# IceTTTb/NopeSAC

Measured on AMD Instinct MI355X. Metric: image-pairs/sec (480x640, K=32 hyp), higher is better.
Workload: dtype bf16; 1 GPU; configs/inference_mp3d.yaml, 32 synthetic 480x640 pairs/GPU/step, ResNet-50 + pyramids in bfloat16, head GEMMs bf16 operands with f32 accumulate / residual stream / LayerNorm / softmax, K=32 matched planes forced (m mean 32.0), nq=50; pairs_per_gpu=32, global_batch=32, K=32, parallelism=pair-sharded dp1, rccl_ranks=1, batches_in_flight_per_gpu=4, hip_graph=False, steps_per_all_gather=8, routing_entries_loaded=45, routing_entries_measured_now=0, nonfinite_outputs=0

## Files before the change

nopesac_amd/csrc/conv_forms.h:

```cpp
#pragma once
#include <initializer_list>

#include "common.h"

namespace nps {

constexpr int P8_SK_MAX_TILES = 4096;

struct ConvCall {
    int x_dt, w_dt, out_dt;
    int B, H, W, Cin, Cout, KH, KW, stride, pad;
    long long x_cs, y_cs, r_cs;
    bool batched, has_residual, has_scale, has_bias;
    int act;
    bool aligned, entry;

    static long long fdiv(long long a, long long b) { return a / b - ((a % b != 0 && ((a < 0) != (b < 0))) ? 1 : 0); }
    long long OH() const { return fdiv(H + 2ll * pad - KH, stride) + 1; }
    long long OW() const { return fdiv(W + 2ll * pad - KW, stride) + 1; }
    long long M() const { return B * OH() * OW(); }
    long long K() const { return (long long)KH * KW * Cin; }
    long long tiles(int bm, int bn) const { return -fdiv(-M(), bm) * (Cout / bn); }
};

static inline bool conv_aligned(std::initializer_list<const void*> ptrs) {
    for (const void* q : ptrs)
        if ((uintptr_t)q % 16 != 0) return false;
    return true;
}

#define NPS_CHECK_CONV(name, expr)                  \
    do {                                            \
        const char* why__ = (expr);                 \
        NPS_CHECK_ARG(!why__, name ": %s", why__);  \
    } while (0)


static inline const char* conv_call_refusal(const ConvCall& c) {
    if (!(c.B > 0 && c.H > 0 && c.W > 0 && c.Cin > 0 && c.Cout > 0 && c.KH > 0 && c.KW > 0 && c.stride > 0 && c.pad >= 0)) return "bad dims";
    if (c.OH() <= 0 || c.OW() <= 0) return "empty output";
    if (c.out_dt != NPS_DT_F32 && c.out_dt != NPS_DT_BF16 && c.out_dt != NPS_DT_FP8) return "bad out_dt";
    if (c.x_cs < c.Cin || c.y_cs < c.Cout || (c.has_residual && c.r_cs < c.Cout)) return "channel stride smaller than channel count";
    if ((c.act & 0xff) > NPS_ACT_SIGMOID) return "bad act";
    return nullptr;
}

static inline const char* conv_dma_refusal(const ConvCall& c, int cout_tile) {
    const int eb = c.x_dt == NPS_DT_FP8 ? 1 : 2;
    if ((c.x_dt != NPS_DT_BF16 && c.x_dt != NPS_DT_FP8) || c.w_dt != c.x_dt || c.batched) return "needs bf16 (or fp8) x and w, shared weights";
    if (c.Cin % 64 != 0 || c.Cout % cout_tile != 0) return cout_tile == 256 ? "needs Cin % 64 == 0 and Cout % 256 == 0" : "needs Cin % 64 == 0 and Cout % 128 == 0";
    if (c.KH * c.KW > 32) return "more than 32 taps";
    if (c.x_cs % (16 / eb) != 0) return "x_cstride must be a multiple of 16 bytes";
    if (((long long)c.B * c.H * c.W + (long long)c.pad * c.W + c.pad) * c.x_cs * eb >= (1ll << 31)) return "input larger than 2 GB";
    return nullptr;
}

static inline const char* conv_idx24_refusal(const ConvCall& c) {
    if ((long long)c.B * c.H * c.W >= (1 << 23) || c.x_cs >= (1 << 24) || c.K() >= (1 << 24)) return "pixel count / strides beyond the 24-bit index math of this kernel";
    if (c.Cout * c.K() * 2 >= (1ll << 31)) return "weights larger than 2 GB";
    return nullptr;
}

static inline const char* conv_bfrag_refusal(const ConvCall& c) {
    if (const char* why = conv_dma_refusal(c, 128)) return why;
    if (c.act & ~(0xff | NPS_ACT_RES_AFTER)) return "unsupported act flags";
    if (c.entry && c.out_dt == NPS_DT_FP8 && (c.has_residual || c.y_cs % 8 != 0 || !c.aligned)) return "fp8 output needs no residual and 8-channel-aligned y / scale / bias";
    return nullptr;
}

static inline const char* conv_halo_refusal(const ConvCall& c) {
    if (const char* why = conv_bfrag_refusal(c)) return why;
    if (c.x_dt != NPS_DT_BF16 || c.out_dt != NPS_DT_BF16) return "bf16 only";
    if (c.KH != 3 || c.KW != 3 || c.stride != 1 || c.pad != 1) return "3x3 / stride 1 / pad 1 only";
    if (c.x_cs != c.Cin || c.y_cs != c.Cout) return "dense channels only";
    if (c.has_residual || !c.has_scale || !c.has_bias || (c.act & ~0xff)) return "y = act(conv * scale + bias) only: scale and bias, no residual";
    return nullptr;
}

static inline const char* conv_p8_refusal(const ConvCall& c) {
    if (const char* why = conv_dma_refusal(c, 256)) return why;
    if (c.x_dt != NPS_DT_BF16) return "bf16 only";
    if (const char* why = conv_idx24_refusal(c)) return why;
    if (c.act & ~(0xff | NPS_ACT_RES_AFTER)) return "unsupported act flags";
    if (c.out_dt != NPS_DT_F32 && c.out_dt != NPS_DT_BF16 && c.out_dt != NPS_DT_FP8) return "bad out_dt";
    const int al = c.out_dt == NPS_DT_F32 ? 4 : 8;
    if (c.has_residual && c.out_dt == NPS_DT_FP8) return "residual with fp8 output";
    if (!c.aligned || c.y_cs % al != 0 || (c.has_residual && c.r_cs % al != 0)) return "every buffer must be 16-byte aligned with 16-byte-aligned y / residual strides";
    if (c.entry && c.M() >= (1 << 23)) return "output pixel count beyond the 24-bit index math of this kernel";
    return nullptr;
}

static inline const char* conv_p8_sk_refusal(const ConvCall& c) {
    if (const char* why = conv_p8_refusal(c)) return why;
    if (c.tiles(256, 256) > P8_SK_MAX_TILES) return "more tiles than the stream-K workspace has arrival counters (use the plain kernel: nothing to balance)";
    return nullptr;
}

static inline const char* conv_p8n_refusal(const ConvCall& c) {
    if (const char* why = conv_dma_refusal(c, 128)) return why;
    if (c.x_dt != NPS_DT_BF16 || c.out_dt != NPS_DT_BF16 || c.has_residual) return "bf16 in / bf16 out, no residual";
    if (const char* why = conv_idx24_refusal(c)) return why;
    if (c.act != NPS_ACT_NONE && c.act != NPS_ACT_RELU && c.act != NPS_ACT_LEAKY) return "act must be none / ReLU / LeakyReLU (no residual forms)";
    if (!c.aligned || c.y_cs % 8 != 0) return "every buffer must be 16-byte aligned with y_cstride % 8 == 0";
    if ((c.M() + 256) * c.y_cs * 2 >= (1ll << 31)) return "output larger than 2 GB";
    return nullptr;
}

static inline const char* conv_p8n_split_refusal(const ConvCall& c, int splits) {
    if (const char* why = conv_p8n_refusal(c)) return why;
    if (splits < 2 || splits > c.Cin / 64 || splits > 16) return "2 <= splits <= min(Cin / 64, 16)";
    if (splits * c.M() * c.Cout * 4 >= (1ll << 31)) return "split-K workspace larger than 2 GB";
    return nullptr;
}


static inline bool conv_p8_sk_offered(const ConvCall& c) { return c.tiles(256, 256) <= 1024 && c.K() >= 512; }

static inline bool conv_p8n_tap_offered(const ConvCall& c) { return c.KH * c.KW > 1; }

static inline int conv_p8n_split_slices(const ConvCall& c) {
    const long long tiles = c.Cout % 128 == 0 ? c.tiles(256, 128) : 0;
    if (tiles == 0) return 0;
    long long s = ConvCall::fdiv(256, tiles);
    if (s > c.Cin / 64) s = c.Cin / 64;
    return (int)(s > 8 ? 8 : s);
}
static inline bool conv_p8n_split_offered(const ConvCall& c, int splits) { return c.K() >= 4096 && splits >= 2; }

}
```

nopesac_amd/csrc/conv_p8_tile.h:

```cpp
#pragma once
#include "conv_common.h"

namespace nps {

template <int K>
struct IC { static constexpr int value = K; };

typedef unsigned int u32x4 __attribute__((ext_vector_type(4)));

constexpr unsigned P8_OOB = 0xFFFFFF00u;

struct P8TileWalk {
    int xcd, slot, run_begin, run_end, stride;
    __device__ __forceinline__ explicit P8TileWalk(int units) {
        const int nx = (int)gridDim.x < 8 ? (int)gridDim.x : 8;
        xcd = blockIdx.x % 8; slot = blockIdx.x / 8;
        const int tq = units / nx, tr = units % nx;
        run_begin = xcd < tr ? xcd * (tq + 1) : tr * (tq + 1) + (xcd - tr) * tq;
        run_end = run_begin + tq + (xcd < tr ? 1 : 0);
        stride = ((int)gridDim.x - xcd + 7) / 8;
    }
};

__device__ __forceinline__ __amdgpu_buffer_rsrc_t p8_x_rsrc(const ConvParams& p) {
    const long long padb = ((long long)p.pad * p.W + p.pad) * p.x_cs * 2;
    return __builtin_amdgcn_make_buffer_rsrc((void*)((const char*)p.x - padb), 0, (int)(((long long)p.B * p.H * p.W * p.x_cs) * 2 + padb), 0x00020000);
}
__device__ __forceinline__ __amdgpu_buffer_rsrc_t p8_w_rsrc(const ConvParams& p) {
    return __builtin_amdgcn_make_buffer_rsrc((void*)p.w, 0, (int)((long long)p.N * p.K * 2), 0x00020000);
}
__device__ __forceinline__ __amdgpu_buffer_rsrc_t p8_rows_rsrc(const void* base, const ConvParams& p, long long cs, bool on = true) {
    return __builtin_amdgcn_make_buffer_rsrc((void*)base, 0, on ? (int)((((long long)p.M - 1) * cs + p.N) * 2) : 0, 0x00020000);
}

__device__ __forceinline__ void p8_divmod(int a, int d, float rcp, int& q, int& r) {
    q = (int)((float)a * rcp);
    r = a - __mul24(q, d);
    if (r < 0) { --q; r += d; }
    if (r >= d) { ++q; r -= d; }
}

template <int BK>
struct P8KCursor {
    int tap, kw, c0;
    unsigned tapoff, k0b;
    unsigned kw_step, kh_step;
    __device__ __forceinline__ explicit P8KCursor(const ConvParams& p)
        : kw_step((unsigned)p.x_cs * 2u), kh_step((unsigned)(p.W - p.KW) * (unsigned)p.x_cs * 2u) {}
    __device__ __forceinline__ void reset(int c_begin) {
        tap = 0; kw = 0; c0 = c_begin; tapoff = 0u; k0b = (unsigned)c_begin * 2u;
    }
    __device__ __forceinline__ void advance(const ConvParams& p) {
        if (p.force == 0) {
            k0b += BK * 2;
            c0 += BK;
            if (c0 >= p.Cin) {
                c0 = 0; ++tap; ++kw;
                tapoff += kw_step;
                if (kw == p.KW) { kw = 0; tapoff += kh_step; }
            }
        } else {
            ++tap; ++kw;
            k0b += (unsigned)p.Cin * 2u;
            tapoff += kw_step;
            if (kw == p.KW) { kw = 0; tapoff += kh_step; }
            if (tap == p.KH * p.KW) {
                tap = 0; kw = 0; tapoff = 0u;
                c0 += BK;
                k0b = (unsigned)c0 * 2u;
            }
        }
    }
    __device__ __forceinline__ void set_cursor(const ConvParams& p, int kt) {
        const int ntaps = p.KH * p.KW;
        int t, c;
        if (p.force == 0) { const int per = p.Cin / BK; t = kt / per; c = (kt - t * per) * BK; }
        else { const int cs = kt / ntaps; t = kt - cs * ntaps; c = cs * BK; }
        const int kh = t / p.KW;
        tap = t; kw = t - kh * p.KW; c0 = c;
        tapoff = (unsigned)(kh * p.W + kw) * (unsigned)p.x_cs * 2u;
        k0b = (unsigned)(t * p.Cin + c) * 2u;
    }
};

template <int BM, int ROWB, int TAB_OFF>
struct P8Rows {
    static_assert(BM == 256 && ROWB == 128, "two pixel halves of two 64-row DMA groups, 128-byte rows");
    unsigned coff[2][2], voff[2][2], mask[2][2];
    float rcp_rpb, rcp_ow;
    __device__ __forceinline__ void init(const ConvParams& p, int wave, int lane) {
        rcp_rpb = 1.0f / (float)p.rows_per_b; rcp_ow = 1.0f / (float)p.OW;
#pragma unroll
        for (int h = 0; h < 2; ++h)
#pragma unroll
            for (int j = 0; j < 2; ++j) {
                const int pr = j * 128 + h * 64 + wave * 8 + (lane >> 3);
                coff[h][j] = (unsigned)((lane & 7) ^ ((pr >> 1) & 7)) * 16u;
            }
    }
    __device__ __forceinline__ void set_tile(unsigned char* lds, const ConvParams& p, int m0, int tid, int wave, int lane) {
        uint2* rowtab = reinterpret_cast<uint2*>(lds + TAB_OFF);
        if (tid < BM) {
            const int m = m0 + tid;
            uint2 e = make_uint2(0u, 0u);
            if (m < p.M) {
                int b, rem, oh, ow;
                p8_divmod(m, p.rows_per_b, rcp_rpb, b, rem);
                p8_divmod(rem, p.OW, rcp_ow, oh, ow);
                const int ih0 = __mul24(oh, p.stride) - p.pad, iw0 = __mul24(ow, p.stride) - p.pad;
                const unsigned pix = __umul24(__umul24((unsigned)b, (unsigned)p.H) + (unsigned)(ih0 + p.pad), (unsigned)p.W) + (unsigned)(iw0 + p.pad);
                unsigned colbits = 0u;
                for (int kw = 0; kw < p.KW; ++kw) colbits |= ((unsigned)(iw0 + kw) < (unsigned)p.W ? 1u : 0u) << kw;
                unsigned mk = 0u;
                for (int kh = 0; kh < p.KH; ++kh)
                    if ((unsigned)(ih0 + kh) < (unsigned)p.H) mk |= colbits << __mul24(kh, p.KW);
                e = make_uint2(__umul24(pix, (unsigned)p.x_cs) * 2u, mk);
            }
            rowtab[tid] = e;
        }
        NPS_LDS_SYNC();
#pragma unroll
        for (int h = 0; h < 2; ++h)
#pragma unroll
            for (int j = 0; j < 2; ++j) {
                const uint2 e = rowtab[j * 128 + h * 64 + wave * 8 + (lane >> 3)];
                voff[h][j] = e.x + coff[h][j];
                mask[h][j] = e.y;
            }
    }
    template <int BK>
    __device__ __forceinline__ void stage_a(const __amdgpu_buffer_rsrc_t& xsrc, unsigned char* buf, int h, int wave, const P8KCursor<BK>& cur) const {
        const unsigned soff = cur.tapoff + (unsigned)cur.c0 * 2u;
#pragma unroll
        for (int j = 0; j < 2; ++j) {
            const unsigned vo = ((mask[h][j] >> cur.tap) & 1u) ? voff[h][j] : P8_OOB;
            __builtin_amdgcn_raw_ptr_buffer_load_lds(xsrc, (lptr_t)(buf + (j * 128 + h * 64 + wave * 8) * ROWB), 16, vo, soff, 0, 0);
        }
    }
};

}
```

nopesac_amd/csrc/conv_p8n.hip:

```cpp
#include "conv_forms.h"
#include "conv_p8_tile.h"

namespace nps {

constexpr int N8_BM = 256, N8_BN = 128, N8_BK = 64, N8_ROWB = 128;
constexpr int N8_A_BYTES = N8_BM * N8_ROWB, N8_B_BYTES = N8_BN * N8_ROWB, N8_STAGE = N8_A_BYTES + N8_B_BYTES;
constexpr int N8_NSTAGE = 3;
constexpr int N8_ELD16 = N8_BN + 8;
constexpr int N8_EPI_OFF = 2 * N8_STAGE;
constexpr int N8_TAB_OFF = N8_NSTAGE * N8_STAGE;
constexpr int N8_LDS = N8_TAB_OFF + N8_BM * 8;

struct N8EpiRegs {
    float sc[4][4], bs[4][4];
};

template <int ACT, bool SPLIT = false>
__global__ __launch_bounds__(512) void conv_igemm_p8n_kernel(const ConvParams p) {
#if defined(__HIP_DEVICE_COMPILE__)
    __shared__ __attribute__((aligned(1024))) unsigned char lds[N8_LDS];
    const int tid = threadIdx.x, lane = tid & 63;
    const int wave = __builtin_amdgcn_readfirstlane(tid >> 6);
    const int wr = wave >> 2, wc = wave & 3;

    const P8TileWalk walk(p.tiles_m * p.tiles_n * (SPLIT ? p.ksplit : 1));
    int tile = walk.run_begin + walk.slot;
    if (tile >= walk.run_end) return;

    const __amdgpu_buffer_rsrc_t xsrc = p8_x_rsrc(p), wsrc = p8_w_rsrc(p), ry = p8_rows_rsrc(p.y, p, p.y_cs);
    P8Rows<N8_BM, N8_ROWB, N8_TAB_OFF> rows;
    P8KCursor<N8_BK> kc(p);
    rows.init(p, wave, lane);
    unsigned b_voff[2], b_base[2];
#pragma unroll
    for (int j = 0; j < 2; ++j) {
        const int br = (wave * 2 + j) * 8 + (lane >> 3);
        b_base[j] = (__umul24((unsigned)br, (unsigned)p.K) + (unsigned)((lane & 7) ^ ((br >> 1) & 7)) * 8u) * 2u;
    }
    int m0 = 0, n0 = 0;
    const int ntaps = p.KH * p.KW;
    int nk = p.K / N8_BK;
    int ks = 0;
    auto set_tile = [&](int t) {
        int c_begin = 0;
        if constexpr (SPLIT) {
            const int tt = t / p.ksplit, ngroups = p.Cin / N8_BK;
            ks = t - tt * p.ksplit;
            c_begin = (ks * ngroups) / p.ksplit;
            nk = (((ks + 1) * ngroups) / p.ksplit - c_begin) * ntaps;
            c_begin *= N8_BK;
            t = tt;
        }
        m0 = (t / p.tiles_n) * N8_BM;
        n0 = (t % p.tiles_n) * N8_BN;
        rows.set_tile(lds, p, m0, tid, wave, lane);
        const unsigned nb = __umul24((unsigned)n0, (unsigned)p.K) * 2u;
#pragma unroll
        for (int j = 0; j < 2; ++j) b_voff[j] = b_base[j] + nb;
        kc.reset(c_begin);
    };
    auto stage_a = [&](unsigned char* buf, int h) { rows.stage_a(xsrc, buf, h, wave, kc); };
    auto stage_b = [&](unsigned char* buf) {
#pragma unroll
        for (int j = 0; j < 2; ++j)
            __builtin_amdgcn_raw_ptr_buffer_load_lds(wsrc, (lptr_t)(buf + N8_A_BYTES + ((wave * 2 + j) * 8) * N8_ROWB), 16, b_voff[j], kc.k0b, 0, 0);
    };
    auto stage_first = [&]() {
        stage_a(lds, 0); stage_b(lds); stage_a(lds, 1);
        kc.advance(p);
        if (nk > 1) {
            stage_a(lds + N8_STAGE, 0); stage_b(lds + N8_STAGE); stage_a(lds + N8_STAGE, 1);
            kc.advance(p);
        }
    };

    const int sw = (lane >> 1) & 7;
    const int a_row_off = (wr * 128 + (lane & 31)) * N8_ROWB;
    const int b_row_off = N8_A_BYTES + (wc * 32 + (lane & 31)) * N8_ROWB;
    int so[4];
#pragma unroll
    for (int ks = 0; ks < 4; ++ks) so[ks] = ((2 * ks + (lane >> 5)) ^ sw) * 16;

    set_tile(tile);
    stage_first();
    bool first = true;
    while (true) {
        f32x16 acc[4];
#pragma unroll
        for (int i = 0; i < 4; ++i)
#pragma unroll
            for (int r = 0; r < 16; ++r) acc[i][r] = 0.f;
        bf16x8 af[2][4], bfr[4];
        if (first) {
            if (nk > 1) asm volatile("s_waitcnt vmcnt(8)" ::: "memory");
            else asm volatile("s_waitcnt vmcnt(2)" ::: "memory");
        }
        __builtin_amdgcn_s_barrier();
        asm volatile("" ::: "memory");
        if (wr == 1) {
            __builtin_amdgcn_s_setprio(1);
            __builtin_amdgcn_s_barrier();
        }
        auto ktile = [&](auto SLOTC, int t) {
            constexpr int SLOT = decltype(SLOTC)::value;
            unsigned char* sb = lds + SLOT * N8_STAGE;
            unsigned char* fb = lds + ((SLOT + 2) % N8_NSTAGE) * N8_STAGE;
            const bool has1 = t + 1 < nk, has2 = t + 2 < nk;
            auto load_a = [&](int mi) {
#pragma unroll
                for (int i = 0; i < 2; ++i)
#pragma unroll
                    for (int ks = 0; ks < 4; ++ks)
                        af[i][ks] = *(const bf16x8*)(sb + a_row_off + (mi * 64 + i * 32) * N8_ROWB + so[ks]);
            };
            auto mfma_phase = [&](auto MIC) {
                constexpr int MI = decltype(MIC)::value;
#pragma unroll
                for (int ks = 0; ks < 4; ++ks)
#pragma unroll
                    for (int i = 0; i < 2; ++i)
                        acc[MI * 2 + i] = __builtin_amdgcn_mfma_f32_32x32x16_bf16(bfr[ks], af[i][ks], acc[MI * 2 + i], 0, 0, 0);
            };
#pragma unroll
            for (int ks = 0; ks < 4; ++ks) bfr[ks] = *(const bf16x8*)(sb + b_row_off + so[ks]);
            load_a(0);
            if (has2) {
                stage_a(fb, 0);
                stage_b(fb);
                asm volatile("s_waitcnt vmcnt(10)" ::: "memory");
            } else if (has1) {
                asm volatile("s_waitcnt vmcnt(6)" ::: "memory");
            } else {
                asm volatile("s_waitcnt vmcnt(0)" ::: "memory");
            }
            NPS_PHASE_BAR();
            mfma_phase(IC<0>{});
            NPS_PHASE_BAR();
            load_a(1);
            if (has2) {
                stage_a(fb, 1);
                kc.advance(p);
                asm volatile("s_waitcnt vmcnt(8)" ::: "memory");
            } else if (has1) {
                asm volatile("s_waitcnt vmcnt(2)" ::: "memory");
            }
            NPS_PHASE_BAR();
            mfma_phase(IC<1>{});
            NPS_PHASE_BAR();
        };
        {
            int t = 0;
            for (; t + 2 < nk; t += 3) {
                ktile(IC<0>{}, t);
                ktile(IC<1>{}, t + 1);
                ktile(IC<2>{}, t + 2);
            }
            if (t < nk) ktile(IC<0>{}, t);
            if (t + 1 < nk) ktile(IC<1>{}, t + 1);
        }
        if (wr == 0) __builtin_amdgcn_s_barrier();
        else __builtin_amdgcn_s_setprio(0);
        NPS_LDS_SYNC();

        const int cur_m0 = m0, cur_n0 = n0, cur_ks = ks;
        const int next = tile + walk.stride;
        const bool more = next < walk.run_end;
        if constexpr (SPLIT) {
            if (more) { set_tile(next); stage_first(); }
            __builtin_amdgcn_sched_barrier(0);
            const __amdgpu_buffer_rsrc_t rws = __builtin_amdgcn_make_buffer_rsrc(p.sk_ws, 0, p.sk_ws_bytes, 0x00020000);
#pragma unroll
            for (int a = 0; a < 4; ++a) {
                const unsigned m = (unsigned)(cur_m0 + wr * 128 + a * 32 + (lane & 31));
                const unsigned row = ((unsigned)cur_ks * (unsigned)p.M + m) * (unsigned)p.N + (unsigned)(cur_n0 + wc * 32 + 4 * (lane >> 5));
#pragma unroll
                for (int q = 0; q < 4; ++q) {
                    const f32x4 v = {acc[a][4 * q], acc[a][4 * q + 1], acc[a][4 * q + 2], acc[a][4 * q + 3]};
                    const unsigned off = m < (unsigned)p.M ? (row + 8u * q) * 4u : P8_OOB;
                    __builtin_amdgcn_raw_buffer_store_b128(__builtin_bit_cast(u32x4, v), rws, (int)off, 0, 0);
                }
            }
            if (more) asm volatile("s_waitcnt vmcnt(16)" ::: "memory");
            if (!more) break;
            tile = next;
            first = false;
            continue;
        }
        N8EpiRegs R;
#pragma unroll
        for (int q = 0; q < 4; ++q) {
            const int n = cur_n0 + wc * 32 + 8 * q + 4 * (lane >> 5);
            f32x4 s4 = {1.f, 1.f, 1.f, 1.f}, b4 = {0.f, 0.f, 0.f, 0.f};
            if (p.scale) s4 = *(const f32x4*)(p.scale + n);
            if (p.bias) b4 = *(const f32x4*)(p.bias + n);
#pragma unroll
            for (int e = 0; e < 4; ++e) { R.sc[q][e] = s4[e]; R.bs[q][e] = b4[e]; }
        }
        if (more) {
            set_tile(next);
#pragma unroll
            for (int q = 0; q < 4; ++q)
#pragma unroll
                for (int e = 0; e < 4; ++e) asm volatile("" :: "v"(R.sc[q][e]), "v"(R.bs[q][e]));
            stage_first();
        }
        {
            bf16_t* epi = reinterpret_cast<bf16_t*>(lds + N8_EPI_OFF);
            const int c8 = tid & 15, rg = tid >> 4;
            auto do_pass = [&](auto PASSC) {
                constexpr int pass = decltype(PASSC)::value;
#pragma unroll
                for (int q = 0; q < 4; ++q) {
                    float v[4];
#pragma unroll
                    for (int e = 0; e < 4; ++e) {
                        float t = acc[pass][4 * q + e] * R.sc[q][e];
                        t += R.bs[q][e];
                        t += 0.f;
                        if (ACT == NPS_ACT_RELU) t = t > 0.f ? t : 0.f;
                        else if (ACT == NPS_ACT_LEAKY) t = t > 0.f ? t : 0.01f * t;
                        v[e] = t;
                    }
                    const uint2 o = make_uint2(f32x2_to_bf16x2(v[0], v[1]), f32x2_to_bf16x2(v[2], v[3]));
                    *(uint2*)(epi + (wr * 32 + (lane & 31)) * N8_ELD16 + wc * 32 + 8 * q + 4 * (lane >> 5)) = o;
                }
                if constexpr (pass == 3) {
                    if (more) asm volatile("s_waitcnt vmcnt(6)" ::: "memory");
                }
                NPS_LDS_SYNC();
                u32x4 o[2];
#pragma unroll
                for (int it = 0; it < 2; ++it) o[it] = *(const u32x4*)(epi + (it * 32 + rg) * N8_ELD16 + c8 * 8);
#pragma unroll
                for (int it = 0; it < 2; ++it) {
                    const unsigned m = (unsigned)(cur_m0 + it * 128 + pass * 32 + rg);
                    __builtin_amdgcn_raw_buffer_store_b128(o[it], ry, (int)((m * (unsigned)p.y_cs + (unsigned)(cur_n0 + c8 * 8)) * 2u), 0, 0);
                }
                NPS_LDS_SYNC();
            };
            do_pass(IC<0>{});
            do_pass(IC<1>{});
            do_pass(IC<2>{});
            do_pass(IC<3>{});
        }
        if (!more) break;
        tile = next;
        first = false;
    }
#endif
}

__global__ __launch_bounds__(256) void p8n_split_reduce_kernel(const float* __restrict__ ws, int splits, int M, int N, const float* __restrict__ scale,
                                                               const float* __restrict__ bias, bf16_t* __restrict__ y, long long y_cs, int act) {
    const long long i = (long long)blockIdx.x * 256 + threadIdx.x, per_row = N / 8;
    if (i >= (long long)M * per_row) return;
    const long long m = i / per_row;
    const int n = (int)(i - m * per_row) * 8;
    const float* src = ws + m * N + n;
    f32x4 a = *reinterpret_cast<const f32x4*>(src), b = *reinterpret_cast<const f32x4*>(src + 4);
    for (int s = 1; s < splits; ++s) {
        const float* q = src + (long long)s * M * N;
        const f32x4 c = *reinterpret_cast<const f32x4*>(q), d = *reinterpret_cast<const f32x4*>(q + 4);
#pragma unroll
        for (int e = 0; e < 4; ++e) { a[e] += c[e]; b[e] += d[e]; }
    }
    f32x4 s0 = {1.f, 1.f, 1.f, 1.f}, s1 = s0, b0 = {0.f, 0.f, 0.f, 0.f}, b1 = b0;
    if (scale) { s0 = *reinterpret_cast<const f32x4*>(scale + n); s1 = *reinterpret_cast<const f32x4*>(scale + n + 4); }
    if (bias) { b0 = *reinterpret_cast<const f32x4*>(bias + n); b1 = *reinterpret_cast<const f32x4*>(bias + n + 4); }
    float v[8];
#pragma unroll
    for (int e = 0; e < 4; ++e) {
        v[e] = a[e] * s0[e];
        v[e] += b0[e];
        v[4 + e] = b[e] * s1[e];
        v[4 + e] += b1[e];
    }
    us8 o;
#pragma unroll
    for (int e = 0; e < 8; ++e) {
        float t = v[e] + 0.f;
        if (act == NPS_ACT_RELU) t = t > 0.f ? t : 0.f;
        else if (act == NPS_ACT_LEAKY) t = t > 0.f ? t : 0.01f * t;
        o[e] = f32_to_bf16(t);
    }
    *reinterpret_cast<us8*>(y + m * y_cs + n) = o;
}

}

extern "C" int64_t nopesac_conv2d_p8n_splitk_workspace_bytes(int splits, int64_t M, int Cout) {
    return splits > 0 && M > 0 && Cout > 0 ? (int64_t)splits * M * Cout * 4 : 0;
}

static int p8n_launch(const void* x, const void* w, const float* scale, const float* bias, void* y, int B, int H, int W,
                      int Cin, int Cout, int KH, int KW, int stride, int pad, int64_t x_cstride, int64_t y_cstride, int act,
                      int variant, int splits, void* workspace, int64_t workspace_bytes, void* stream) {
    using namespace nps;
    NPS_CHECK_ARG(x && w && y, "conv2d_p8n: null pointer");
    const ConvCall c = {NPS_DT_BF16, NPS_DT_BF16, NPS_DT_BF16, B, H, W, Cin, Cout, KH, KW, stride, pad, x_cstride, y_cstride, 0, false, false,
                        scale != nullptr, bias != nullptr, act, conv_aligned({x, w, y, scale, bias}), true};
    NPS_CHECK_CONV("conv2d_p8n", conv_call_refusal(c));
    NPS_CHECK_CONV("conv2d_p8n", splits > 1 ? conv_p8n_split_refusal(c, splits) : conv_p8n_refusal(c));
    const int kmajor = (variant >> 5) & 1;
    const int grid_cap = variant >> 8;
    NPS_CHECK_ARG((variant & 0xdf) == 0, "conv2d_p8n: variant must be 0 (+ 32: channel-major K order, + (n << 8): grid cap)");
    ConvParams p;
    conv_params_fill(p, x, w, scale, bias, nullptr, y, B, H, W, Cin, Cout, KH, KW, stride, pad, x_cstride, y_cstride, 0, act, 0, NPS_DT_BF16);
    p.force = kmajor;
    p.tiles_m = (p.M + N8_BM - 1) / N8_BM;
    p.tiles_n = p.N / N8_BN;
    const hipStream_t st = (hipStream_t)stream;
    if (splits > 1) {
        const long long need = nopesac_conv2d_p8n_splitk_workspace_bytes(splits, p.M, p.N);
        NPS_CHECK_ARG(kmajor, "conv2d_p8n_splitk: variant must carry + 32 (channel-major K order)");
        NPS_CHECK_ARG(workspace && ((uintptr_t)workspace % 16 == 0) && workspace_bytes >= need,
                      "conv2d_p8n_splitk: workspace of splits * M * N * 4 bytes, 16-byte aligned");
        p.ksplit = splits; p.sk_ws = workspace; p.sk_ws_bytes = (int)need;
        const dim3 grid(conv_persistent_grid(grid_cap, p.tiles_m * p.tiles_n * splits));
        hipLaunchKernelGGL((conv_igemm_p8n_kernel<NPS_ACT_NONE, true>), grid, dim3(512), 0, st, p);
        const long long items = (long long)p.M * (p.N / 8);
        hipLaunchKernelGGL(p8n_split_reduce_kernel, dim3((unsigned)((items + 255) / 256)), dim3(256), 0, st, (const float*)workspace, splits, p.M, p.N,
                           scale, bias, (bf16_t*)y, (long long)y_cstride, act);
        NPS_LAUNCH_RET();
    }
    const dim3 grid(conv_persistent_grid(grid_cap, p.tiles_m * p.tiles_n));
    if (act == NPS_ACT_RELU) hipLaunchKernelGGL((conv_igemm_p8n_kernel<NPS_ACT_RELU>), grid, dim3(512), 0, st, p);
    else if (act == NPS_ACT_LEAKY) hipLaunchKernelGGL((conv_igemm_p8n_kernel<NPS_ACT_LEAKY>), grid, dim3(512), 0, st, p);
    else hipLaunchKernelGGL((conv_igemm_p8n_kernel<NPS_ACT_NONE>), grid, dim3(512), 0, st, p);
    NPS_LAUNCH_RET();
}

extern "C" int nopesac_conv2d_nhwc_p8n(const void* x, const void* w, const float* scale, const float* bias, void* y, int B, int H, int W,
                                       int Cin, int Cout, int KH, int KW, int stride, int pad, int64_t x_cstride, int64_t y_cstride, int act,
                                       int variant, void* stream) {
    return p8n_launch(x, w, scale, bias, y, B, H, W, Cin, Cout, KH, KW, stride, pad, x_cstride, y_cstride, act, variant, 1, nullptr, 0, stream);
}

extern "C" int nopesac_conv2d_nhwc_p8n_splitk(const void* x, const void* w, const float* scale, const float* bias, void* y, int B, int H, int W,
                                              int Cin, int Cout, int KH, int KW, int stride, int pad, int64_t x_cstride, int64_t y_cstride,
                                              int act, int variant, int splits, void* workspace, int64_t workspace_bytes, void* stream) {
    NPS_CHECK_ARG(splits >= 2, "conv2d_p8n_splitk: splits >= 2");
    return p8n_launch(x, w, scale, bias, y, B, H, W, Cin, Cout, KH, KW, stride, pad, x_cstride, y_cstride, act, variant, splits, workspace,
                      workspace_bytes, stream);
}
```

Measured before the change: 4096 pairs/s.

## Share one staged A row block across the three kw taps in 3x3 p8n conv

For 3x3 stride-1 pad-1 convolutions in channel-major K order, the p8n implicit-GEMM kernel now stages a 264-row A block (the tile plus one halo row on each side) once per kh and channel chunk. The three kw taps read it at row offsets of 0, +1 and +2, with precomputed per-lane LDS offsets that redirect edge columns to a zero region. This removes two thirds of the global-to-LDS A loads for these convs. In exchange it adds a new LDS layout, a hand-tuned waitcnt schedule and an nk%3 structure. The path is on by default for matching shapes and can be disabled with variant bit 64.

```diff
diff --git a/nopesac_amd/csrc/conv_forms.h b/nopesac_amd/csrc/conv_forms.h
--- a/nopesac_amd/csrc/conv_forms.h
+++ b/nopesac_amd/csrc/conv_forms.h
@@ -106,6 +106,10 @@
     return nullptr;
 }
 
+static inline bool conv_p8n_shared_kw(const ConvCall& c, bool channel_major) {
+    return channel_major && c.KH == 3 && c.KW == 3 && c.stride == 1 && c.pad == 1;
+}
+
 static inline const char* conv_p8n_split_refusal(const ConvCall& c, int splits) {
     if (const char* why = conv_p8n_refusal(c)) return why;
     if (splits < 2 || splits > c.Cin / 64 || splits > 16) return "2 <= splits <= min(Cin / 64, 16)";
diff --git a/nopesac_amd/csrc/conv_p8_tile.h b/nopesac_amd/csrc/conv_p8_tile.h
--- a/nopesac_amd/csrc/conv_p8_tile.h
+++ b/nopesac_amd/csrc/conv_p8_tile.h
@@ -139,4 +139,54 @@
     }
 };
 
+template <int ROWB, int TAB_OFF>
+struct P8RowsKw {
+    static_assert(ROWB == 128, "128-byte rows");
+    static constexpr int ROWS = 264, USED = 258;
+    unsigned coff[5], voff[5], rmask;
+    unsigned keep;
+    float rcp_rpb, rcp_ow;
+    __device__ __forceinline__ static int piece_row(int j, int wave, int lane) { return j < 4 ? j * 64 + wave * 8 + (lane >> 3) : 256 + wave; }
+    __device__ __forceinline__ void init(const ConvParams& p, int wave, int lane) {
+        rcp_rpb = 1.0f / (float)p.rows_per_b; rcp_ow = 1.0f / (float)p.OW;
+#pragma unroll
+        for (int j = 0; j < 5; ++j) coff[j] = (unsigned)((lane & 7) ^ ((piece_row(j, wave, lane) >> 1) & 7)) * 16u;
+    }
+    __device__ __forceinline__ void set_tile(unsigned char* lds, const ConvParams& p, int m0, int tid, int wave, int lane, int wr) {
+        uint2* rowtab = reinterpret_cast<uint2*>(lds + TAB_OFF);
+        if (tid < ROWS) {
+            const int c = m0 + tid - 1;
+            uint2 e = make_uint2(0u, 0u);
+            if (tid < USED && c >= 0 && c < p.M) {
+                int b, rem, h, w;
+                p8_divmod(c, p.rows_per_b, rcp_rpb, b, rem);
+                p8_divmod(rem, p.OW, rcp_ow, h, w);
+                unsigned bits = 2u | (h > 0 ? 1u : 0u) | (h + 1 < p.H ? 4u : 0u);
+                bits |= (w == 0 ? 8u : 0u) | (w == p.W - 1 ? 16u : 0u);
+                e = make_uint2(__umul24((unsigned)(c + 1), (unsigned)p.x_cs) * 2u, bits);
+            }
+            rowtab[tid] = e;
+        }
+        NPS_LDS_SYNC();
+        rmask = 0u;
+#pragma unroll
+        for (int j = 0; j < 5; ++j) {
+            const uint2 e = rowtab[piece_row(j, wave, lane)];
+            voff[j] = e.x + coff[j];
+            rmask |= (e.y & 7u) << (3 * j);
+        }
+        keep = 0u;
+#pragma unroll
+        for (int a = 0; a < 4; ++a) {
+            const unsigned f = rowtab[wr * 128 + a * 32 + (lane & 31) + 1].y;
+            keep |= (((f >> 3) & 1u) ^ 1u) << (2 * a) | (((f >> 4) & 1u) ^ 1u) << (2 * a + 1);
+        }
+    }
+    __device__ __forceinline__ void stage_a(const __amdgpu_buffer_rsrc_t& xsrc, unsigned char* buf, int j, int wave, int lane, int kh, unsigned soff) const {
+        const unsigned vo = ((rmask >> (3 * j + kh)) & 1u) ? voff[j] : P8_OOB;
+        if (j < 4) __builtin_amdgcn_raw_ptr_buffer_load_lds(xsrc, (lptr_t)(buf + (j * 64 + wave * 8) * ROWB), 16, vo, soff, 0, 0);
+        else if ((lane >> 3) == wave) __builtin_amdgcn_raw_ptr_buffer_load_lds(xsrc, (lptr_t)(buf + 256 * ROWB), 16, vo, soff, 0, 0);
+    }
+};
+
 }
diff --git a/nopesac_amd/csrc/conv_p8n.hip b/nopesac_amd/csrc/conv_p8n.hip
--- a/nopesac_amd/csrc/conv_p8n.hip
+++ b/nopesac_amd/csrc/conv_p8n.hip
@@ -1,5 +1,7 @@
 #include "conv_forms.h"
 #include "conv_p8_tile.h"
+
+#include <type_traits>
 
 namespace nps {
 
@@ -11,14 +13,21 @@
 constexpr int N8_TAB_OFF = N8_NSTAGE * N8_STAGE;
 constexpr int N8_LDS = N8_TAB_OFF + N8_BM * 8;
 
+constexpr int KW_ROWS = 264, KW_A_BYTES = KW_ROWS * N8_ROWB;
+constexpr int KW_B_OFF = 2 * KW_A_BYTES;
+constexpr int KW_EPI_OFF = KW_A_BYTES;
+constexpr int KW_TAB_OFF = KW_B_OFF + N8_NSTAGE * N8_B_BYTES;
+constexpr int KW_LDS = KW_TAB_OFF + KW_ROWS * 8;
+static_assert(64 * N8_ELD16 * 2 <= KW_A_BYTES, "a 64-row epilogue pass fits an A buffer");
+
 struct N8EpiRegs {
     float sc[4][4], bs[4][4];
 };
 
-template <int ACT, bool SPLIT = false>
+template <int ACT, bool SPLIT = false, bool SKW = false>
 __global__ __launch_bounds__(512) void conv_igemm_p8n_kernel(const ConvParams p) {
 #if defined(__HIP_DEVICE_COMPILE__)
-    __shared__ __attribute__((aligned(1024))) unsigned char lds[N8_LDS];
+    __shared__ __attribute__((aligned(1024))) unsigned char lds[SKW ? KW_LDS : N8_LDS];
     const int tid = threadIdx.x, lane = tid & 63;
     const int wave = __builtin_amdgcn_readfirstlane(tid >> 6);
     const int wr = wave >> 2, wc = wave & 3;
@@ -28,9 +37,12 @@
     if (tile >= walk.run_end) return;
 
     const __amdgpu_buffer_rsrc_t xsrc = p8_x_rsrc(p), wsrc = p8_w_rsrc(p), ry = p8_rows_rsrc(p.y, p, p.y_cs);
-    P8Rows<N8_BM, N8_ROWB, N8_TAB_OFF> rows;
+    std::conditional_t<SKW, P8RowsKw<N8_ROWB, KW_TAB_OFF>, P8Rows<N8_BM, N8_ROWB, N8_TAB_OFF>> rows;
     P8KCursor<N8_BK> kc(p);
     rows.init(p, wave, lane);
+    int a_kh = 0;
+    unsigned a_soff = 0u, a_c2 = 0u;
+    const unsigned a_kh_step = (unsigned)p.W * (unsigned)p.x_cs * 2u;
     unsigned b_voff[2], b_base[2];
 #pragma unroll
     for (int j = 0; j < 2; ++j) {
@@ -53,19 +65,42 @@
         }
         m0 = (t / p.tiles_n) * N8_BM;
         n0 = (t % p.tiles_n) * N8_BN;
-        rows.set_tile(lds, p, m0, tid, wave, lane);
+        if constexpr (SKW) rows.set_tile(lds, p, m0, tid, wave, lane, wr);
+        else rows.set_tile(lds, p, m0, tid, wave, lane);
         const unsigned nb = __umul24((unsigned)n0, (unsigned)p.K) * 2u;
 #pragma unroll
         for (int j = 0; j < 2; ++j) b_voff[j] = b_base[j] + nb;
         kc.reset(c_begin);
-    };
-    auto stage_a = [&](unsigned char* buf, int h) { rows.stage_a(xsrc, buf, h, wave, kc); };
+        a_kh = 0; a_c2 = (unsigned)c_begin * 2u; a_soff = a_c2;
+    };
+
+    auto stage_a = [&](unsigned char* buf, int h) {
+        if constexpr (SKW) rows.stage_a(xsrc, buf, h, wave, lane, a_kh, a_soff);
+        else rows.stage_a(xsrc, buf, h, wave, kc);
+    };
+    auto advance_a = [&]() {
+        ++a_kh; a_soff += a_kh_step;
+        if (a_kh == 3) { a_kh = 0; a_c2 += N8_BK * 2; a_soff = a_c2; }
+    };
+    auto stage_bk = [&](int slot) {
+#pragma unroll
+        for (int j = 0; j < 2; ++j)
+            __builtin_amdgcn_raw_ptr_buffer_load_lds(wsrc, (lptr_t)(lds + KW_B_OFF + slot * N8_B_BYTES + ((wave * 2 + j) * 8) * N8_ROWB), 16, b_voff[j], kc.k0b, 0, 0);
+        kc.advance(p);
+    };
     auto stage_b = [&](unsigned char* buf) {
 #pragma unroll
         for (int j = 0; j < 2; ++j)
             __builtin_amdgcn_raw_ptr_buffer_load_lds(wsrc, (lptr_t)(buf + N8_A_BYTES + ((wave * 2 + j) * 8) * N8_ROWB), 16, b_voff[j], kc.k0b, 0, 0);
     };
     auto stage_first = [&]() {
+        if constexpr (SKW) {
+#pragma unroll
+            for (int j = 0; j < 5; ++j) stage_a(lds, j);
+            advance_a();
+            stage_bk(0); stage_bk(1);
+            return;
+        }
         stage_a(lds, 0); stage_b(lds); stage_a(lds, 1);
         kc.advance(p);
         if (nk > 1) {
@@ -80,8 +115,27 @@
     int so[4];
 #pragma unroll
     for (int ks = 0; ks < 4; ++ks) so[ks] = ((2 * ks + (lane >> 5)) ^ sw) * 16;
+    int so1[4], aoff[2][4][4];
+#pragma unroll
+    for (int ks = 0; ks < 4; ++ks) so1[ks] = ((2 * ks + (lane >> 5)) ^ ((((lane & 31) + 1) >> 1) & 7)) * 16;
+    auto set_aoff = [&]() {
+        if constexpr (SKW) {
+#pragma unroll
+            for (int k2 = 0; k2 < 2; ++k2)
+#pragma unroll
+                for (int a = 0; a < 4; ++a) {
+                    const bool keep = (rows.keep >> (2 * a + k2)) & 1u;
+#pragma unroll
+                    for (int ks = 0; ks < 4; ++ks) {
+                        const int in_row = a_row_off + (a * 32 + 2 * k2) * N8_ROWB + ((2 * ks + (lane >> 5)) ^ ((((lane & 31) + 2 * k2) >> 1) & 7)) * 16;
+                        aoff[k2][a][ks] = keep ? in_row : P8RowsKw<N8_ROWB, KW_TAB_OFF>::USED * N8_ROWB + ks * 16;
+                    }
+                }
+        }
+    };
 
     set_tile(tile);
+    set_aoff();
     stage_first();
     bool first = true;
     while (true) {
@@ -92,7 +146,8 @@
             for (int r = 0; r < 16; ++r) acc[i][r] = 0.f;
         bf16x8 af[2][4], bfr[4];
         if (first) {
-            if (nk > 1) asm volatile("s_waitcnt vmcnt(8)" ::: "memory");
+            if constexpr (SKW) asm volatile("s_waitcnt vmcnt(2)" ::: "memory");
+            else if (nk > 1) asm volatile("s_waitcnt vmcnt(8)" ::: "memory");
             else asm volatile("s_waitcnt vmcnt(2)" ::: "memory");
         }
         __builtin_amdgcn_s_barrier();
@@ -101,62 +156,125 @@
             __builtin_amdgcn_s_setprio(1);
             __builtin_amdgcn_s_barrier();
         }
-        auto ktile = [&](auto SLOTC, int t) {
-            constexpr int SLOT = decltype(SLOTC)::value;
-            unsigned char* sb = lds + SLOT * N8_STAGE;
-            unsigned char* fb = lds + ((SLOT + 2) % N8_NSTAGE) * N8_STAGE;
-            const bool has1 = t + 1 < nk, has2 = t + 2 < nk;
-            auto load_a = [&](int mi) {
-#pragma unroll
-                for (int i = 0; i < 2; ++i)
+        if constexpr (SKW) {
+            auto triple = [&](auto ABC, const bool has_next) {
+                constexpr int AB = decltype(ABC)::value;
+                unsigned char* ab = lds + AB * KW_A_BYTES;
+                unsigned char* an = lds + (AB ^ 1) * KW_A_BYTES;
+                auto ktile = [&](auto KWC) {
+                    constexpr int KW = decltype(KWC)::value;
+                    auto load_a = [&](int mi) {
+#pragma unroll
+                        for (int i = 0; i < 2; ++i)
+#pragma unroll
+                            for (int ks = 0; ks < 4; ++ks)
+                                af[i][ks] = KW == 1 ? *(const bf16x8*)(ab + a_row_off + (mi * 64 + i * 32 + 1) * N8_ROWB + so1[ks])
+                                                    : *(const bf16x8*)(ab + aoff[KW >> 1][mi * 2 + i][ks]);
+                    };
+                    auto mfma_phase = [&](auto MIC) {
+                        constexpr int MI = decltype(MIC)::value;
+#pragma unroll
+                        for (int ks = 0; ks < 4; ++ks)
+#pragma unroll
+                            for (int i = 0; i < 2; ++i)
+                                acc[MI * 2 + i] = __builtin_amdgcn_mfma_f32_32x32x16_bf16(bfr[ks], af[i][ks], acc[MI * 2 + i], 0, 0, 0);
+                    };
+#pragma unroll
+                    for (int ks = 0; ks < 4; ++ks) bfr[ks] = *(const bf16x8*)(lds + KW_B_OFF + KW * N8_B_BYTES + b_row_off - N8_A_BYTES + so[ks]);
+                    load_a(0);
+                    if (KW == 1 && has_next) {
+                        stage_a(an, 3); stage_a(an, 4);
+                        advance_a();
+                    }
+                    if (KW == 0 || has_next) stage_bk((KW + 2) % 3);
+                    NPS_PHASE_BAR();
+                    mfma_phase(IC<0>{});
+                    NPS_PHASE_BAR();
+                    load_a(1);
+                    if constexpr (KW == 0) {
+                        if (has_next) {
+                            stage_a(an, 0); stage_a(an, 1); stage_a(an, 2);
+                            asm volatile("s_waitcnt vmcnt(5)" ::: "memory");
+                        } else {
+                            asm volatile("s_waitcnt vmcnt(2)" ::: "memory");
+                        }
+                    } else if constexpr (KW == 1) {
+                        if (has_next) asm volatile("s_waitcnt vmcnt(7)" ::: "memory");
+                        else asm volatile("s_waitcnt vmcnt(0)" ::: "memory");
+                    } else {
+                        if (has_next) asm volatile("s_waitcnt vmcnt(2)" ::: "memory");
+                    }
+                    NPS_PHASE_BAR();
+                    mfma_phase(IC<1>{});
+                    NPS_PHASE_BAR();
+                };
+                ktile(IC<0>{});
+                ktile(IC<1>{});
+                ktile(IC<2>{});
+            };
+            const int nt = nk / 3;
+            for (int T = 0; T < nt; T += 2) {
+                triple(IC<0>{}, T + 1 < nt);
+                if (T + 1 < nt) triple(IC<1>{}, T + 2 < nt);
+            }
+        } else {
+            auto ktile = [&](auto SLOTC, int t) {
+                constexpr int SLOT = decltype(SLOTC)::value;
+                unsigned char* sb = lds + SLOT * N8_STAGE;
+                unsigned char* fb = lds + ((SLOT + 2) % N8_NSTAGE) * N8_STAGE;
+                const bool has1 = t + 1 < nk, has2 = t + 2 < nk;
+                auto load_a = [&](int mi) {
+#pragma unroll
+                    for (int i = 0; i < 2; ++i)
+#pragma unroll
+                        for (int ks = 0; ks < 4; ++ks)
+                            af[i][ks] = *(const bf16x8*)(sb + a_row_off + (mi * 64 + i * 32) * N8_ROWB + so[ks]);
+                };
+                auto mfma_phase = [&](auto MIC) {
+                    constexpr int MI = decltype(MIC)::value;
 #pragma unroll
                     for (int ks = 0; ks < 4; ++ks)
-                        af[i][ks] = *(const bf16x8*)(sb + a_row_off + (mi * 64 + i * 32) * N8_ROWB + so[ks]);
+#pragma unroll
+                        for (int i = 0; i < 2; ++i)
+                            acc[MI * 2 + i] = __builtin_amdgcn_mfma_f32_32x32x16_bf16(bfr[ks], af[i][ks], acc[MI * 2 + i], 0, 0, 0);
+                };
+#pragma unroll
+                for (int ks = 0; ks < 4; ++ks) bfr[ks] = *(const bf16x8*)(sb + b_row_off + so[ks]);
+                load_a(0);
+                if (has2) {
+                    stage_a(fb, 0);
+                    stage_b(fb);
+                    asm volatile("s_waitcnt vmcnt(10)" ::: "memory");
+                } else if (has1) {
+                    asm volatile("s_waitcnt vmcnt(6)" ::: "memory");
+                } else {
+                    asm volatile("s_waitcnt vmcnt(0)" ::: "memory");
+                }
+                NPS_PHASE_BAR();
+                mfma_phase(IC<0>{});
+                NPS_PHASE_BAR();
+                load_a(1);
+                if (has2) {
+                    stage_a(fb, 1);
+                    kc.advance(p);
+                    asm volatile("s_waitcnt vmcnt(8)" ::: "memory");
+                } else if (has1) {
+                    asm volatile("s_waitcnt vmcnt(2)" ::: "memory");
+                }
+                NPS_PHASE_BAR();
+                mfma_phase(IC<1>{});
+                NPS_PHASE_BAR();
             };
-            auto mfma_phase = [&](auto MIC) {
-                constexpr int MI = decltype(MIC)::value;
-#pragma unroll
-                for (int ks = 0; ks < 4; ++ks)
-#pragma unroll
-                    for (int i = 0; i < 2; ++i)
-                        acc[MI * 2 + i] = __builtin_amdgcn_mfma_f32_32x32x16_bf16(bfr[ks], af[i][ks], acc[MI * 2 + i], 0, 0, 0);
-            };
-#pragma unroll
-            for (int ks = 0; ks < 4; ++ks) bfr[ks] = *(const bf16x8*)(sb + b_row_off + so[ks]);
-            load_a(0);
-            if (has2) {
-                stage_a(fb, 0);
-                stage_b(fb);
-                asm volatile("s_waitcnt vmcnt(10)" ::: "memory");
-            } else if (has1) {
-                asm volatile("s_waitcnt vmcnt(6)" ::: "memory");
-            } else {
-                asm volatile("s_waitcnt vmcnt(0)" ::: "memory");
+            {
+                int t = 0;
+                for (; t + 2 < nk; t += 3) {
+                    ktile(IC<0>{}, t);
+                    ktile(IC<1>{}, t + 1);
+                    ktile(IC<2>{}, t + 2);
+                }
+                if (t < nk) ktile(IC<0>{}, t);
+                if (t + 1 < nk) ktile(IC<1>{}, t + 1);
             }
-            NPS_PHASE_BAR();
-            mfma_phase(IC<0>{});
-            NPS_PHASE_BAR();
-            load_a(1);
-            if (has2) {
-                stage_a(fb, 1);
-                kc.advance(p);
-                asm volatile("s_waitcnt vmcnt(8)" ::: "memory");
-            } else if (has1) {
-                asm volatile("s_waitcnt vmcnt(2)" ::: "memory");
-            }
-            NPS_PHASE_BAR();
-            mfma_phase(IC<1>{});
-            NPS_PHASE_BAR();
-        };
-        {
-            int t = 0;
-            for (; t + 2 < nk; t += 3) {
-                ktile(IC<0>{}, t);
-                ktile(IC<1>{}, t + 1);
-                ktile(IC<2>{}, t + 2);
-            }
-            if (t < nk) ktile(IC<0>{}, t);
-            if (t + 1 < nk) ktile(IC<1>{}, t + 1);
         }
         if (wr == 0) __builtin_amdgcn_s_barrier();
         else __builtin_amdgcn_s_setprio(0);
@@ -166,7 +284,11 @@
         const int next = tile + walk.stride;
         const bool more = next < walk.run_end;
         if constexpr (SPLIT) {
-            if (more) { set_tile(next); stage_first(); }
+            if (more) {
+                set_tile(next);
+                set_aoff();
+                stage_first();
+            }
             __builtin_amdgcn_sched_barrier(0);
             const __amdgpu_buffer_rsrc_t rws = __builtin_amdgcn_make_buffer_rsrc(p.sk_ws, 0, p.sk_ws_bytes, 0x00020000);
 #pragma unroll
@@ -202,10 +324,11 @@
             for (int q = 0; q < 4; ++q)
 #pragma unroll
                 for (int e = 0; e < 4; ++e) asm volatile("" :: "v"(R.sc[q][e]), "v"(R.bs[q][e]));
+            set_aoff();
             stage_first();
         }
         {
-            bf16_t* epi = reinterpret_cast<bf16_t*>(lds + N8_EPI_OFF);
+            bf16_t* epi = reinterpret_cast<bf16_t*>(lds + (SKW ? KW_EPI_OFF : N8_EPI_OFF));
             const int c8 = tid & 15, rg = tid >> 4;
             auto do_pass = [&](auto PASSC) {
                 constexpr int pass = decltype(PASSC)::value;
@@ -303,7 +426,8 @@
     NPS_CHECK_CONV("conv2d_p8n", splits > 1 ? conv_p8n_split_refusal(c, splits) : conv_p8n_refusal(c));
     const int kmajor = (variant >> 5) & 1;
     const int grid_cap = variant >> 8;
-    NPS_CHECK_ARG((variant & 0xdf) == 0, "conv2d_p8n: variant must be 0 (+ 32: channel-major K order, + (n << 8): grid cap)");
+    NPS_CHECK_ARG((variant & 0x9f) == 0, "conv2d_p8n: variant must be 0 (+ 32: channel-major K order, + 64: per-tap K loop, + (n << 8): grid cap)");
+    const bool skw = !(variant & 64) && conv_p8n_shared_kw(c, kmajor != 0);
     ConvParams p;
     conv_params_fill(p, x, w, scale, bias, nullptr, y, B, H, W, Cin, Cout, KH, KW, stride, pad, x_cstride, y_cstride, 0, act, 0, NPS_DT_BF16);
     p.force = kmajor;
@@ -317,13 +441,20 @@
                       "conv2d_p8n_splitk: workspace of splits * M * N * 4 bytes, 16-byte aligned");
         p.ksplit = splits; p.sk_ws = workspace; p.sk_ws_bytes = (int)need;
         const dim3 grid(conv_persistent_grid(grid_cap, p.tiles_m * p.tiles_n * splits));
-        hipLaunchKernelGGL((conv_igemm_p8n_kernel<NPS_ACT_NONE, true>), grid, dim3(512), 0, st, p);
+        if (skw) hipLaunchKernelGGL((conv_igemm_p8n_kernel<NPS_ACT_NONE, true, true>), grid, dim3(512), 0, st, p);
+        else hipLaunchKernelGGL((conv_igemm_p8n_kernel<NPS_ACT_NONE, true>), grid, dim3(512), 0, st, p);
         const long long items = (long long)p.M * (p.N / 8);
         hipLaunchKernelGGL(p8n_split_reduce_kernel, dim3((unsigned)((items + 255) / 256)), dim3(256), 0, st, (const float*)workspace, splits, p.M, p.N,
                            scale, bias, (bf16_t*)y, (long long)y_cstride, act);
         NPS_LAUNCH_RET();
     }
     const dim3 grid(conv_persistent_grid(grid_cap, p.tiles_m * p.tiles_n));
+    if (skw) {
+        if (act == NPS_ACT_RELU) hipLaunchKernelGGL((conv_igemm_p8n_kernel<NPS_ACT_RELU, false, true>), grid, dim3(512), 0, st, p);
+        else if (act == NPS_ACT_LEAKY) hipLaunchKernelGGL((conv_igemm_p8n_kernel<NPS_ACT_LEAKY, false, true>), grid, dim3(512), 0, st, p);
+        else hipLaunchKernelGGL((conv_igemm_p8n_kernel<NPS_ACT_NONE, false, true>), grid, dim3(512), 0, st, p);
+        NPS_LAUNCH_RET();
+    }
     if (act == NPS_ACT_RELU) hipLaunchKernelGGL((conv_igemm_p8n_kernel<NPS_ACT_RELU>), grid, dim3(512), 0, st, p);
     else if (act == NPS_ACT_LEAKY) hipLaunchKernelGGL((conv_igemm_p8n_kernel<NPS_ACT_LEAKY>), grid, dim3(512), 0, st, p);
     else hipLaunchKernelGGL((conv_igemm_p8n_kernel<NPS_ACT_NONE>), grid, dim3(512), 0, st, p);
```

New measurement: 4120 pairs/s (median of 6 runs). About the same (+0.6%).
